# rogermm14/eonerf_code

Hardware: AMD Instinct MI355X
Metric: train rays/sec on JAX_068 (4096 rays x 128 samples) (higher is better)
Workload: dtype bf16

## Files before the change

eonerf_code_amd/csrc/eonerf_bwd_pipe.hip:

```cpp
#include "eonerf_common.h"
#include "eonerf_kernels.h"
#include "eonerf_ambient_dev.h"

namespace {

constexpr int NT = 512;
constexpr int TS = PIPE_TS;
constexpr int IMG_B = 16 * 1024;
constexpr int SLOT_B = 2 * IMG_B;
#ifndef EO_PIPE_STAMPS
#define EO_PIPE_STAMPS 0
#endif
constexpr int NSLOT = 4, DEPTH = 3, DDEPTH = 2;
static_assert(DDEPTH < DEPTH && DEPTH < NSLOT, "prefetch distances (the counted waits of Cnt assume DDEPTH < DEPTH)");
EO_DEV int slot_of(int k) { return k & (NSLOT - 1); }
constexpr uint32_t RING_USE = PIPE_RING;
constexpr int N_DMA = 4;
constexpr int CTRL_B = 64;
constexpr int SMEM_B = NSLOT * SLOT_B + CTRL_B;
constexpr int AUX_SC1 = 16, AUX_NT = 2;
constexpr unsigned long long WATCHDOG_TICKS = 30000000ull;

typedef __attribute__((address_space(1))) unsigned int gu32;

EO_DEV int wg_swz16(int row, int chunk) { return (chunk ^ ((row >> 2) & 3)) * 16; }

constexpr int NST = 2;
template <bool CTRL, bool ORDB> struct Cnt {
    static constexpr int C = (CTRL ? 4 : 0) + NST + N_DMA;
    static constexpr int TOP = ORDB ? C : N_DMA / 2 + (DDEPTH - 1) * C;
    static constexpr int TOP_CTRL = NST + N_DMA;
};

struct Stage {
    int pipe, st, n_k;
    bool has_in;
    int x_row;
    const uint8_t* in_lin;
    uint8_t* out_lin;
    bool local;
};

template <bool CTRL, int MODE, bool ORDB = false>
EO_DEV void run_stage(const BwdPipeArgs& a, const Stage& S, uint8_t* smem, int tid) {
    constexpr bool HAS_OUT = MODE == 0 || MODE == 1;
    constexpr bool RING_OUT = MODE == 0;
    typedef PBf16 P;
    typedef P::U U;
    const int lane = tid & 63, wave = __builtin_amdgcn_readfirstlane(tid >> 6), h = lane >> 5, c = lane & 31;
    int* const ctl = reinterpret_cast<int*>(smem + NSLOT * SLOT_B);
    const int n_k = S.n_k;

    U wt[16];
    {
        const uint8_t* src = a.wt + ((size_t)(S.st * 8 + wave) * 16) * 1024 + lane * 16;
#pragma unroll
        for (int kg = 0; kg < 16; ++kg) wt[kg] = *reinterpret_cast<const U*>(src + kg * 1024);
        __builtin_amdgcn_s_waitcnt(0x0F70);
    }
    f32x16 dw[8];
#pragma unroll
    for (int j = 0; j < 8; ++j) dw[j] = zero_acc();
    float db = 0.f;

    const size_t n_tiles = (size_t)a.p_pad / TS;
    const int n_edges = a.n_stages - 1;
    const uint8_t* x_base = reinterpret_cast<const uint8_t*>(a.act) + (size_t)S.x_row * n_tiles * SEG_B;
    uint8_t* const ring_in = a.rings + (size_t)(S.pipe * n_edges + (S.st - 1)) * PIPE_RING * IMG_B;
    uint8_t* const ring_out = a.rings + (size_t)(S.pipe * n_edges + S.st) * PIPE_RING * IMG_B;
    gu32* const f_in = (gu32*)(a.flags + (size_t)(S.pipe * n_edges + (S.st - 1)) * 64);
    gu32* const f_out = (gu32*)(a.flags + (size_t)(S.pipe * n_edges + S.st) * 64);
    gu32* const my_scratch = (gu32*)(a.scratch_word + (size_t)(S.pipe * a.n_stages + S.st) * 32);

    uint8_t* const grd_blk = S.out_lin;
    const uint8_t* const in_blk = S.in_lin;

    int x_voff[2];
#pragma unroll
    for (int j = 0; j < 2; ++j) {
        const int row = 32 * wave + 16 * j + (lane >> 2);
        x_voff[j] = row * SEG_B + (((lane & 3) ^ ((row >> 2) & 3)) * 16);
    }
    const uint32_t lin_stride = (uint32_t)a.n_pipes * IMG_B;
    const bool in_ring = S.has_in && !in_blk;
    const uint8_t* const d_base = !S.has_in ? a.dy_in + (size_t)S.pipe * IMG_B : (in_blk ? in_blk + (size_t)S.pipe * IMG_B : ring_in);
    const uint32_t d_mask = in_ring ? RING_USE - 1 : 0x7fffffffu, d_mul = in_ring ? IMG_B : lin_stride;
    const __amdgpu_buffer_rsrc_t rs_d = __builtin_amdgcn_make_buffer_rsrc(const_cast<uint8_t*>(d_base), 0, -1, 0x00020000);
    const __amdgpu_buffer_rsrc_t rs_x = __builtin_amdgcn_make_buffer_rsrc(const_cast<uint8_t*>(x_base) + (size_t)S.pipe * 256 * SEG_B, 0, -1, 0x00020000);
    const __amdgpu_buffer_rsrc_t rs_o = __builtin_amdgcn_make_buffer_rsrc(MODE == 0 ? ring_out : grd_blk + (size_t)S.pipe * IMG_B, 0, -1, 0x00020000);
    const int v_dy = lane * 16 + (2 * wave) * 1024;
    struct Dma { uint32_t so_d, so_x; uint8_t *slot, *slot_d; };
    auto dma_prep = [&](int kx, int kd) {
        Dma d;
        d.slot = smem + slot_of(kx) * SLOT_B;
        d.slot_d = smem + slot_of(kd) * SLOT_B;
        d.so_d = ((uint32_t)kd & d_mask) * d_mul;
        d.so_x = (uint32_t)kx * lin_stride;
        return d;
    };
    auto dma_piece = [&](const Dma& d, int i) {
        if (i < 2) {
            if (S.has_in)
                __builtin_amdgcn_raw_ptr_buffer_load_lds(rs_d, (__attribute__((address_space(3))) void*)(d.slot_d + (2 * wave + i) * 1024), 16,
                                                         lane * 16 + (2 * wave + i) * 1024, d.so_d, 0, AUX_SC1);
            else
                __builtin_amdgcn_raw_ptr_buffer_load_lds(rs_d, (__attribute__((address_space(3))) void*)(d.slot_d + (2 * wave + i) * 1024), 16,
                                                         lane * 16 + (2 * wave + i) * 1024, d.so_d, 0, AUX_NT);
        } else {
            __builtin_amdgcn_raw_ptr_buffer_load_lds(rs_x, (__attribute__((address_space(3))) void*)(d.slot + IMG_B + (32 * wave + 16 * (i - 2)) * SEG_B), 16,
                                                     x_voff[i - 2], d.so_x, 0, AUX_NT);
        }
    };
    auto issue = [&](int k, bool with_dy) {
        const Dma d = dma_prep(k, k);
#pragma unroll
        for (int i = 0; i < N_DMA; ++i) if (with_dy || i >= 2) dma_piece(d, i);
    };

    const int g4 = lane >> 4, i16 = lane & 15, qq = i16 >> 2, pp = i16 & 3;
    const int tr_off = (2 * wave + (g4 & 1)) * 1024 + ((pp & 1) * 32 + 8 * (g4 >> 1) + qq) * 16 + (pp >> 1) * 8;
    const int xb_off0 = IMG_B + c * SEG_B + wg_swz16(c, h), xb_off1 = IMG_B + c * SEG_B + wg_swz16(c, 2 + h);
    int xm_off[4];
#pragma unroll
    for (int q = 0; q < 4; ++q) {
        const int f0 = 32 * wave + 8 * q + 4 * (g4 >> 1);
        xm_off[q] = IMG_B + (f0 + qq) * SEG_B + wg_swz16(f0, 2 * (g4 & 1) + (pp >> 1)) + (pp & 1) * 8;
    }

    int known_head = S.has_in ? 0 : 0x7fffffff, known_tail = RING_OUT ? 0 : 0x7fffffff;
    unsigned ph = 0, pt = 0;
    auto poll_sync = [&](gu32* word) -> int {
        return (int)__hip_atomic_load(word, __ATOMIC_RELAXED, __HIP_MEMORY_SCOPE_AGENT);
    };
    bool aborted = false;
    auto wait_for = [&](gu32* word, int need, int& known) {
        if (known >= need || aborted) return;
        const unsigned long long t0 = __builtin_amdgcn_s_memrealtime();
        for (unsigned it = 0;; ++it) {
            known = poll_sync(word);
            if (known >= need) return;
            __builtin_amdgcn_s_sleep(2);
            const bool expired = __builtin_amdgcn_s_memrealtime() - t0 > WATCHDOG_TICKS;
            const bool other = (it & 63) == 63 && __hip_atomic_load(a.error, __ATOMIC_RELAXED, __HIP_MEMORY_SCOPE_AGENT) != 0;
            if (expired || other) {
                if (lane == 0) { if (expired) atomicOr(a.error, 1 << (S.st & 7)); ctl[0] = 1; }
                asm volatile("s_waitcnt lgkmcnt(0)" ::: "memory");
                aborted = true;
                return;
            }
        }
    };

    const bool stamp = EO_PIPE_STAMPS && a.stamps != nullptr;
    auto clk = [&]() -> uint32_t { return (uint32_t)__builtin_amdgcn_s_memtime(); };
    uint32_t t_slow = 0, t_top = 0, t_bar = 0, t_dx = 0, t_is = 0, t_dw = 0, n_slow = 0;
    const uint32_t t_begin = stamp ? clk() : 0;

    if (CTRL && S.has_in) wait_for(f_in, n_k < DDEPTH ? n_k : DDEPTH, known_head);
    if (CTRL) asm volatile("s_waitcnt vmcnt(0) lgkmcnt(0)" ::: "memory");
    __syncthreads();
    if (ctl[0]) return;
#pragma unroll
    for (int d = 0; d < DEPTH; ++d) issue(d < n_k ? d : n_k - 1, d < DDEPTH);
    asm volatile("s_waitcnt vmcnt(%0)" ::"n"((DEPTH - 1) * N_DMA - (DEPTH - DDEPTH) * (N_DMA / 2)) : "memory");

    for (int k = 0; k < n_k; ++k) {
        uint8_t* slot = smem + slot_of(k) * SLOT_B;
        const uint32_t tt0 = stamp ? clk() : 0;
        asm volatile("s_waitcnt vmcnt(%0)" ::"n"(CTRL ? Cnt<CTRL, ORDB>::TOP_CTRL : Cnt<CTRL, ORDB>::TOP) : "memory");
        const uint32_t tt1 = stamp ? clk() : 0;
        if (CTRL) {
            asm volatile("" : "+v"(ph), "+v"(pt));
            if (k >= 1) {
                const int vh = __builtin_amdgcn_readfirstlane((int)ph), vt = __builtin_amdgcn_readfirstlane((int)pt);
                if (S.has_in && vh > known_head) known_head = vh;
                if (RING_OUT && vt > known_tail) known_tail = vt;
            }
            const int need_in = k + DDEPTH < n_k ? k + DDEPTH + 1 : n_k;
            const int need_out = k + 1 - RING_USE;
            const uint32_t ts0 = stamp ? clk() : 0;
            const bool slow = (S.has_in && known_head < need_in) || (RING_OUT && known_tail < need_out);
            if (S.has_in && known_head < need_in) wait_for(f_in, need_in, known_head);
            if (RING_OUT && known_tail < need_out) wait_for(f_out + 32, need_out, known_tail);
            if (stamp && slow) { t_slow += clk() - ts0; ++n_slow; }
        }
        asm volatile("s_barrier" ::: "memory");
        const uint32_t tt2 = stamp ? clk() : 0;
        if (stamp) { t_top += tt1 - tt0; t_bar += tt2 - tt1; }
        if ((k & 7) == 0 && ctl[0]) return;
        if (CTRL) {
            if (lane == 0) {
                if (S.has_in) __hip_atomic_store(f_in + 32, (unsigned)(k + 1), __ATOMIC_RELAXED, __HIP_MEMORY_SCOPE_AGENT);
                else __hip_atomic_store(my_scratch, 0u, __ATOMIC_RELAXED, __HIP_MEMORY_SCOPE_AGENT);
                if (HAS_OUT) __hip_atomic_store(f_out, (unsigned)(k > 0 && S.st != a.fault_stage ? k - 1 : 0), __ATOMIC_RELAXED, __HIP_MEMORY_SCOPE_AGENT);
                else __hip_atomic_store((my_scratch + 1), 0u, __ATOMIC_RELAXED, __HIP_MEMORY_SCOPE_AGENT);
            }
            const gu32* a_h = S.has_in ? f_in : my_scratch;
            const gu32* a_t = RING_OUT ? f_out + 32 : my_scratch;
            asm volatile("global_load_dword %0, %2, off sc1\n\tglobal_load_dword %1, %3, off sc1"
                         : "=&v"(ph), "=&v"(pt) : "v"(a_h), "v"(a_t) : "memory");
        }

        auto phase_dx = [&]() {
            f32x16 acc = zero_acc();
            u32x2 xm[4] = {};
            {
                const uint8_t* bp = slot + lane * 16;
                constexpr int WIN = 3;
                U fr[WIN];
#pragma unroll
                for (int d = 0; d < WIN; ++d) fr[d] = lds_unit<P>(bp + d * 1024);
#pragma unroll
                for (int kg = 0; kg < 16; ++kg) {
                    acc = P::mma(wt[kg], fr[kg % WIN], acc);
                    if (kg + WIN < 16) fr[kg % WIN] = lds_unit<P>(bp + (kg + WIN) * 1024);
                    __builtin_amdgcn_sched_barrier(0);
                }
            }
            asm volatile("ds_read_b64_tr_b16 %0, %4\n\t"
                         "ds_read_b64_tr_b16 %1, %5\n\t"
                         "ds_read_b64_tr_b16 %2, %6\n\t"
                         "ds_read_b64_tr_b16 %3, %7\n\t"
                         "s_waitcnt lgkmcnt(0)"
                         : "=&v"(xm[0]), "=&v"(xm[1]), "=&v"(xm[2]), "=&v"(xm[3])
                         : "v"((uint32_t)(uintptr_t)(slot + xm_off[0])), "v"((uint32_t)(uintptr_t)(slot + xm_off[1])),
                           "v"((uint32_t)(uintptr_t)(slot + xm_off[2])), "v"((uint32_t)(uintptr_t)(slot + xm_off[3])) : "memory");
            uint32_t w8[8];
#pragma unroll
            for (int s = 0; s < 8; ++s) {
                uint32_t flags, r;
                const uint32_t xw = xm[s >> 1][s & 1];
                asm("v_pk_min_u16 %0, %1, %2" : "=v"(flags) : "v"(xw), "v"(0x00010001u));
                asm("v_pk_mul_lo_u16 %0, %1, %2" : "=v"(r) : "v"(cvt_pk_bf16(acc[2 * s], acc[2 * s + 1])), "v"(flags));
                w8[s] = r;
            }
            const uint32_t so_o = MODE == 0 ? ((uint32_t)k & (RING_USE - 1)) * IMG_B : (uint32_t)k * lin_stride;
            if (HAS_OUT && S.local) {
                __builtin_amdgcn_raw_buffer_store_b128(u32x4{w8[0], w8[1], w8[2], w8[3]}, rs_o, v_dy, so_o, 0);
                __builtin_amdgcn_raw_buffer_store_b128(u32x4{w8[4], w8[5], w8[6], w8[7]}, rs_o, v_dy + 1024, so_o, 0);
            } else if (HAS_OUT) {
                __builtin_amdgcn_raw_buffer_store_b128(u32x4{w8[0], w8[1], w8[2], w8[3]}, rs_o, v_dy, so_o, AUX_SC1);
                __builtin_amdgcn_raw_buffer_store_b128(u32x4{w8[4], w8[5], w8[6], w8[7]}, rs_o, v_dy + 1024, so_o, AUX_SC1);
            } else {
                __builtin_amdgcn_raw_buffer_store_b128(u32x4{w8[0], w8[1], w8[2], w8[3]}, rs_o, v_dy, so_o, AUX_NT);
                __builtin_amdgcn_raw_buffer_store_b128(u32x4{w8[4], w8[5], w8[6], w8[7]}, rs_o, v_dy + 1024, so_o, AUX_NT);
            }
        };
        u32x2 ta[2][2] = {};
        auto dw_prefetch = [&]() {
            const uint32_t ra = (uint32_t)(uintptr_t)(slot + tr_off);
            asm volatile("ds_read_b64_tr_b16 %0, %4\n\t"
                         "ds_read_b64_tr_b16 %1, %4 offset:64\n\t"
                         "ds_read_b64_tr_b16 %2, %4 offset:256\n\t"
                         "ds_read_b64_tr_b16 %3, %4 offset:320"
                         : "=&v"(ta[0][0]), "=&v"(ta[0][1]), "=&v"(ta[1][0]), "=&v"(ta[1][1]) : "v"(ra) : "memory");
        };
        auto phase_dw = [&]() {
            asm volatile("s_waitcnt lgkmcnt(0)" : "+v"(ta[0][0]), "+v"(ta[0][1]), "+v"(ta[1][0]), "+v"(ta[1][1]) :: "memory");
#pragma unroll
            for (int ks = 0; ks < 2; ++ks) {
                const U af = __builtin_bit_cast(U, u32x4{ta[ks][0][0], ta[ks][0][1], ta[ks][1][0], ta[ks][1][1]});
                const uint8_t* xb = slot + (ks ? xb_off1 : xb_off0);
                U bf[2];
                bf[0] = lds_unit<P>(xb);
                bf[1] = lds_unit<P>(xb + 2048);
#pragma unroll
                for (int j = 0; j < 8; ++j) {
                    dw[j] = P::mma(af, bf[j & 1], dw[j]);
                    if (j + 2 < 8) bf[j & 1] = lds_unit<P>(xb + (j + 2) * 2048);
                    __builtin_amdgcn_sched_barrier(0);
                }
                const u32x4 av = __builtin_bit_cast(u32x4, af);
#pragma unroll
                for (int e = 0; e < 4; ++e) db += __uint_as_float(av[e] << 16) + __uint_as_float(av[e] & 0xffff0000u);
            }
        };
        const int k_next = k + DEPTH < n_k ? k + DEPTH : n_k - 1;
        const Dma dma = dma_prep(k_next, k + DDEPTH < n_k ? k + DDEPTH : n_k - 1);
        auto issue_block = [&]() {
#pragma unroll
            for (int i = 0; i < N_DMA; ++i) dma_piece(dma, i);
        };
        if (!ORDB) {
            phase_dx();
            const uint32_t tt3 = stamp ? clk() : 0;
            dw_prefetch();
            issue_block();
            const uint32_t tt4 = stamp ? clk() : 0;
            phase_dw();
            if (stamp) { t_dx += tt3 - tt2; t_is += tt4 - tt3; t_dw += clk() - tt4; }
        } else {
            dw_prefetch();
            issue_block();
            const uint32_t tt3 = stamp ? clk() : 0;
            phase_dw();
            const uint32_t tt4 = stamp ? clk() : 0;
            phase_dx();
            if (stamp) { t_is += tt3 - tt2; t_dw += tt4 - tt3; t_dx += clk() - tt4; }
        }
    }
    if (stamp && lane == 0) {
        unsigned long long* o = a.stamps + ((size_t)(S.pipe * a.n_stages + S.st) * 8 + wave) * 16;
        o[0] = clk() - t_begin; o[1] = t_slow; o[2] = t_top; o[3] = t_bar; o[4] = t_dx; o[5] = n_slow; o[6] = (unsigned long long)n_k;
        o[7] = 0; o[8] = t_is; o[9] = 0; o[10] = t_dw;
    }
    asm volatile("s_waitcnt vmcnt(0)" ::: "memory");
    __syncthreads();
    if (CTRL && lane == 0 && HAS_OUT && S.st != a.fault_stage) __hip_atomic_store(f_out, (unsigned)n_k, __ATOMIC_RELAXED, __HIP_MEMORY_SCOPE_AGENT);

    db += __shfl_xor(db, 32, 64);
    if (a.partials) {
        float* pt = a.partials + (size_t)(S.pipe * a.n_stages + S.st) * (256 * 256 + 256);
#pragma unroll
        for (int j = 0; j < 8; ++j)
#pragma unroll
            for (int g = 0; g < 16; ++g) pt[(32 * wave + acc_row(g, h)) * 256 + 32 * j + c] = dw[j][g];
        if (h == 0) pt[256 * 256 + 32 * wave + c] = db;
        return;
    }
    float* dwp = a.d_flat + a.dw_off[S.st];
    float* dbp = a.d_flat + a.db_off[S.st];
    const int ld = a.dw_ld[S.st];
    const int row0 = 32 * wave;
#pragma unroll
    for (int j = 0; j < 8; ++j)
#pragma unroll
        for (int g = 0; g < 16; ++g) atomicAdd(dwp + (size_t)(row0 + acc_row(g, h)) * ld + 32 * j + c, dw[j][g]);
    if (h == 0) atomicAdd(dbp + row0 + c, db);
}

EO_DEV bool take_role(const BwdPipeArgs& a, uint8_t* smem, int tid, Stage& S, int& extra) {
    int* const ctl = reinterpret_cast<int*>(smem + NSLOT * SLOT_B);
    if (tid == 0) {
        ctl[0] = 0; ctl[2] = 0;
        if (!a.xcd_local) ctl[1] = atomicAdd(a.role_counter, 1);
        else {
            const int xcc = (int)(__builtin_amdgcn_s_getreg((3 << 11) | 20) & 7u);
            const int rx = atomicAdd(a.role_counter + 1 + xcc, 1);
// ... 109 lines not shown
```

eonerf_code_amd/csrc/eonerf_enc_pair.hip:

```cpp
#include "eonerf_common.h"
#include "eonerf_kernels.h"

namespace {

constexpr int NT = 512;
constexpr int IMG = 16 * 1024;
constexpr int ENC_B = ENC_SLOTS * SEG_B;
constexpr int SLOT_B = 2 * IMG + ENC_B;
constexpr int NS = 4, DEPTH = NS - 1;
constexpr int N_DMA = 9;
constexpr int GP_F = 4 * 32 * 4;
constexpr int SMEM_B = NS * SLOT_B + 2 * GP_F * (int)sizeof(float);

EO_DEV int swz16(int row, int chunk) { return (chunk ^ ((row >> 2) & 3)) * 16; }

EO_DEV void enc_waves(const EncPairArgs& a, uint8_t* smem, int lane, int wave, int t0, int t1, int n_pts) {
    typedef PBf16 P;
    typedef P::U U;
    const int h = lane >> 5, c = lane & 31;
    const int s_src = wave >> 1, mt = wave & 1;
    U wt[16];
#pragma unroll
    for (int kg = 0; kg < 16; ++kg) wt[kg] = *reinterpret_cast<const U*>(a.wt + ((size_t)((s_src * 2 + mt) * 16 + kg)) * 1024 + lane * 16);
    float* gp_lds = reinterpret_cast<float*>(smem + NS * SLOT_B);
    const float eoff = h ? EO_PI_2_F : 0.0f;
    auto load_pos = [&](int t, float& x, float& y, float& z) {
        const int p = t * 32 + c;
        const bool live = p < n_pts;
        x = live ? a.px[p] : 0.f; y = live ? a.py[p] : 0.f; z = live ? a.pz[p] : 0.f;
    };
    auto finish = [&](int t_prev, int par) {
        const int p = t_prev * 32 + c;
        if (h == 0 && p < n_pts) {
            const f32x4* g = reinterpret_cast<const f32x4*>(gp_lds + par * GP_F);
            f32x4 v = g[c];
#pragma unroll
            for (int w = 1; w < 4; ++w) { const f32x4 u = g[w * 32 + c]; v[0] += u[0]; v[1] += u[1]; v[2] += u[2]; }
            a.g_pos[p] = v[0]; a.g_pos[(size_t)a.p_pad + p] = v[1]; a.g_pos[2 * (size_t)a.p_pad + p] = v[2];
        }
    };
    float x, y, z;
    load_pos(t0, x, y, z);
    for (int t = t0; t < t1; ++t) {
        const int slot = (t - t0) & (NS - 1), par = (t - t0) & 1;
        asm volatile("s_barrier" ::: "memory");
        if (wave == 0 && t > t0) finish(t - 1, par ^ 1);
        const uint8_t* bp = smem + slot * SLOT_B + s_src * IMG + lane * 16;
        f32x16 acc = zero_acc();
        U fr[3];
#pragma unroll
        for (int d = 0; d < 3; ++d) fr[d] = lds_unit<P>(bp + d * 1024);
#pragma unroll
        for (int kg = 0; kg < 16; ++kg) {
            acc = P::mma(wt[kg], fr[kg % 3], acc);
            if (kg + 3 < 16) fr[kg % 3] = lds_unit<P>(bp + (kg + 3) * 1024);
        }
        float gp[3] = {0.f, 0.f, 0.f};
#pragma unroll
        for (int r = 0; r < 16; ++r) {
            const float g = acc[r];
            if (mt == 0 || r < 14) {
                const int q0 = r, q1 = 16 + r;
                const int k = mt ? q1 / 3 : q0 / 3, d = mt ? q1 % 3 : q0 % 3;
                const float cc = d == 0 ? x : (d == 1 ? y : z);
                const float arg = cc * (float)(1 << k) + eoff;
                gp[d] += g * (__cosf(arg) * (float)(1 << k));
            } else if (r == 14) {
                if (h) gp[2] += g; else gp[0] += g;
            } else {
                if (!h) gp[1] += g;
            }
        }
#pragma unroll
        for (int d = 0; d < 3; ++d) gp[d] += __shfl_xor(gp[d], 32, 64);
        if (h == 0) reinterpret_cast<f32x4*>(gp_lds + par * GP_F)[wave * 32 + c] = f32x4{gp[0], gp[1], gp[2], 0.f};
        if (t + 1 < t1) load_pos(t + 1, x, y, z);
    }
    asm volatile("s_barrier" ::: "memory");
    if (wave == 0) finish(t1 - 1, (t1 - 1 - t0) & 1);
}

EO_DEV void dw_waves(const EncPairArgs& a, uint8_t* smem, int lane, int wave, int t0, int t1) {
    typedef PBf16 P;
    typedef P::U U;
    const int h = lane >> 5, c = lane & 31, v = wave - 4;
    const int s_src = v >> 1, mhalf = v & 1;
    const size_t nt = (size_t)a.p_pad / 32;
    const uint8_t* grd = reinterpret_cast<const uint8_t*>(a.grd);
    const __amdgpu_buffer_rsrc_t rs_y0 = __builtin_amdgcn_make_buffer_rsrc(const_cast<uint8_t*>(grd) + (size_t)GRD_ROW_Y0 * nt * SEG_B, 0, -1, 0x00020000);
    const __amdgpu_buffer_rsrc_t rs_y5 = __builtin_amdgcn_make_buffer_rsrc(const_cast<uint8_t*>(grd) + (size_t)(GRD_ROW_Y0 + 5 * 256) * nt * SEG_B, 0, -1, 0x00020000);
    const __amdgpu_buffer_rsrc_t rs_e = __builtin_amdgcn_make_buffer_rsrc(const_cast<uint8_t*>(reinterpret_cast<const uint8_t*>(a.act)) + (size_t)ACT_ROW_ENC * nt * SEG_B, 0, -1, 0x00020000);
    const int enc_row = 16 * v + (lane >> 2);
    const int enc_voff = enc_row * SEG_B + (((lane & 3) ^ ((enc_row >> 2) & 3)) * 16);
    auto issue = [&](int t, int slot) {
        uint8_t* base = smem + slot * SLOT_B;
        const uint32_t so = (uint32_t)t * IMG;
#pragma unroll
        for (int i = 0; i < 4; ++i) {
            __builtin_amdgcn_raw_ptr_buffer_load_lds(rs_y0, (__attribute__((address_space(3))) void*)(base + (4 * v + i) * 1024), 16, lane * 16 + (4 * v + i) * 1024, so, 0, 2);
            __builtin_amdgcn_raw_ptr_buffer_load_lds(rs_y5, (__attribute__((address_space(3))) void*)(base + IMG + (4 * v + i) * 1024), 16, lane * 16 + (4 * v + i) * 1024, so, 0, 2);
        }
        __builtin_amdgcn_raw_ptr_buffer_load_lds(rs_e, (__attribute__((address_space(3))) void*)(base + 2 * IMG + 16 * v * SEG_B), 16, enc_voff, (uint32_t)t * ENC_B, 0, 2);
    };
    f32x16 dw[4][2];
    float dbv[4] = {0.f, 0.f, 0.f, 0.f};
#pragma unroll
    for (int i = 0; i < 4; ++i) { dw[i][0] = zero_acc(); dw[i][1] = zero_acc(); }
    const int g4 = lane >> 4, qq = (lane & 15) >> 2, pp = lane & 3;
    int off_a[4];
#pragma unroll
    for (int i = 0; i < 4; ++i)
        off_a[i] = s_src * IMG + (2 * (4 * mhalf + i) + (g4 & 1)) * 1024 + ((pp & 1) * 32 + 8 * (g4 >> 1) + qq) * 16 + (pp >> 1) * 8;
    int off_b[2][2];
#pragma unroll
    for (int j = 0; j < 2; ++j)
#pragma unroll
        for (int ks = 0; ks < 2; ++ks) { const int row = 32 * j + c; off_b[j][ks] = 2 * IMG + row * SEG_B + swz16(row, 2 * ks + h); }

#pragma unroll
    for (int d = 0; d < DEPTH; ++d) issue(t0 + d < t1 ? t0 + d : t1 - 1, d);
    for (int t = t0; t < t1; ++t) {
        const int slot = (t - t0) & (NS - 1);
        asm volatile("s_waitcnt vmcnt(%0)\n\ts_barrier" ::"n"(N_DMA * (DEPTH - 1)) : "memory");
        issue(t + DEPTH < t1 ? t + DEPTH : t1 - 1, (slot + DEPTH) & (NS - 1));
        const uint8_t* T = smem + slot * SLOT_B;
#pragma unroll
        for (int ks = 0; ks < 2; ++ks) {
            u32x2 ta[8];
            asm volatile("ds_read_b64_tr_b16 %0, %8\n\t"
                         "ds_read_b64_tr_b16 %1, %8 offset:64\n\t"
                         "ds_read_b64_tr_b16 %2, %9\n\t"
                         "ds_read_b64_tr_b16 %3, %9 offset:64\n\t"
                         "ds_read_b64_tr_b16 %4, %10\n\t"
                         "ds_read_b64_tr_b16 %5, %10 offset:64\n\t"
                         "ds_read_b64_tr_b16 %6, %11\n\t"
                         "ds_read_b64_tr_b16 %7, %11 offset:64\n\t"
                         "s_waitcnt lgkmcnt(0)"
                         : "=&v"(ta[0]), "=&v"(ta[1]), "=&v"(ta[2]), "=&v"(ta[3]), "=&v"(ta[4]), "=&v"(ta[5]), "=&v"(ta[6]), "=&v"(ta[7])
                         : "v"((uint32_t)(uintptr_t)(T + off_a[0] + 256 * ks)), "v"((uint32_t)(uintptr_t)(T + off_a[1] + 256 * ks)),
                           "v"((uint32_t)(uintptr_t)(T + off_a[2] + 256 * ks)), "v"((uint32_t)(uintptr_t)(T + off_a[3] + 256 * ks)) : "memory");
            const U b0 = lds_unit<P>(T + off_b[0][ks]), b1 = lds_unit<P>(T + off_b[1][ks]);
#pragma unroll
            for (int i = 0; i < 4; ++i) {
                const u32x4 av = u32x4{ta[2 * i][0], ta[2 * i][1], ta[2 * i + 1][0], ta[2 * i + 1][1]};
                const U af = __builtin_bit_cast(U, av);
                dw[i][0] = P::mma(af, b0, dw[i][0]);
                dw[i][1] = P::mma(af, b1, dw[i][1]);
                if (s_src == 0) {
#pragma unroll
                    for (int e = 0; e < 4; ++e) dbv[i] += __uint_as_float(av[e] << 16) + __uint_as_float(av[e] & 0xffff0000u);
                }
            }
        }
    }
    asm volatile("s_waitcnt vmcnt(0)" ::: "memory");
    float* part = a.part + (size_t)blockIdx.x * ENC_PART_F + (size_t)s_src * 256 * 64;
#pragma unroll
    for (int i = 0; i < 4; ++i)
#pragma unroll
        for (int j = 0; j < 2; ++j)
#pragma unroll
            for (int g = 0; g < 16; ++g) part[((4 * mhalf + i) * 32 + acc_row(g, h)) * 64 + 32 * j + c] = dw[i][j][g];
    if (s_src == 0) {
#pragma unroll
        for (int i = 0; i < 4; ++i) {
            const float sum = dbv[i] + __shfl_xor(dbv[i], 32, 64);
            if (h == 0) a.part[(size_t)blockIdx.x * ENC_PART_F + 2 * 256 * 64 + (4 * mhalf + i) * 32 + c] = sum;
        }
    }
}

__global__ __launch_bounds__(NT) void k_enc_pair(EncPairArgs a) {
    extern __shared__ __attribute__((aligned(16))) uint8_t smem[];
    const int lane = threadIdx.x & 63, wave = __builtin_amdgcn_readfirstlane(threadIdx.x >> 6);
    const int n_pts = *a.n_pts;
    const int n_tiles = (n_pts + 255) / 256 * 8;
    const int t0 = (int)((long long)blockIdx.x * n_tiles / gridDim.x), t1 = (int)((long long)(blockIdx.x + 1) * n_tiles / gridDim.x);
    if (t0 >= t1) {
        for (int i = threadIdx.x; i < ENC_PART_F; i += NT) a.part[(size_t)blockIdx.x * ENC_PART_F + i] = 0.f;
        return;
    }
    if (wave < 4) enc_waves(a, smem, lane, wave, t0, t1, n_pts);
    else dw_waves(a, smem, lane, wave, t0, t1);
}

}

hipError_t eo_launch_enc_pair(const EncPairArgs& a, int n_wg, hipStream_t st) {
    static EoAttrOnce attr;
    {
        const hipError_t e = attr.ensure([&] { return hipFuncSetAttribute(reinterpret_cast<const void*>(&k_enc_pair), hipFuncAttributeMaxDynamicSharedMemorySize, SMEM_B); });
        if (e != hipSuccess) return e;
    }
    hipLaunchKernelGGL(k_enc_pair, dim3(n_wg), dim3(NT), SMEM_B, st, a);
    return hipGetLastError();
}
```

eonerf_code_amd/csrc/eonerf_wgrad_dev.h:

```cpp
#pragma once
#include "eonerf_common.h"
#include "eonerf_kernels.h"
#include <type_traits>

namespace eo_wgrad {

constexpr int WG_NT = 512;
constexpr int MAX_ROWS = 256;
constexpr int ROW_B = SEG_B;
constexpr int OPND_B = MAX_ROWS * ROW_B;
constexpr int SLOT_B = 2 * OPND_B;
constexpr int NS = 4;
constexpr int DEPTH = NS - 1;
constexpr int WMAX = 4, NMAX = 2;
constexpr int AUX_B = 2048;
constexpr int AUX_SIG_WAVE = 7, AUX_EMB_WAVE = 6;

EO_DEV int wg_swz(int row, int chunk) { return (chunk ^ ((row >> 2) & 3)) * 16; }

constexpr int WG_SMEM = NS * SLOT_B + NS * AUX_B + 16;

template <class P>
EO_DEV void wgrad_work(const WgradJobTable& tab, int* queue, float* partials, uint8_t* smem) {
    typedef typename P::U U;
    constexpr int BK = ROW_B / P::ACT_BYTES;
    const int tid = threadIdx.x, lane = tid & 63, wid = __builtin_amdgcn_readfirstlane(tid >> 6), h = lane >> 5, r = lane & 31;
    uint8_t* const lds_aux = smem + NS * SLOT_B;
    int* const lds_item = reinterpret_cast<int*>(smem + NS * SLOT_B + NS * AUX_B);

  for (;;) {
    __syncthreads();
    if (tid == 0) *lds_item = atomicAdd(queue, 1);
    __syncthreads();
    const int item = __builtin_amdgcn_readfirstlane(*lds_item);
    if (item >= tab.items) return;
    int ji = 0;
    while (ji + 1 < tab.n && item >= tab.j[ji + 1].item0) ++ji;
    const WgradJob job = tab.j[ji];
    const int w = item - job.item0, n_slices = job.slices;
    const int n_pts = *job.n_pts;
    const int n_pad = (n_pts + P::TILE - 1) / P::TILE * P::TILE;
    const int steps = n_pad / BK;
    const int s0 = (int)((long long)w * steps / n_slices), s1 = (int)((long long)(w + 1) * steps / n_slices);
    if (s0 >= s1) continue;

    const int wm = job.wm, wn = job.wn, gn = job.gn;
    const bool active = wid < job.gm * gn;
    const int wm_idx = wid / gn, wn_idx = wid % gn;

    int voff_a[2], voff_b[2];
    bool on_a[2], on_b[2];
    int n_dma = 0;
#pragma unroll
    for (int j = 0; j < 2; ++j) {
        const int row = 32 * wid + 16 * j + (lane >> 2);
        const int chunk = (lane & 3) ^ ((row >> 2) & 3);
        const int ra = row < job.m_rows ? row : job.m_rows - 1, rb = row < job.n_rows ? row : job.n_rows - 1;
        voff_a[j] = job.a_units ? (32 * wid + 16 * j) * SEG_B + lane * 16 : ra * SEG_B + chunk * 16;
        voff_b[j] = rb * SEG_B + chunk * 16;
        on_a[j] = 32 * wid + 16 * j < job.m_rows;
        on_b[j] = 32 * wid + 16 * j < job.n_rows;
        n_dma += (on_a[j] ? 1 : 0) + (on_b[j] ? 1 : 0);
    }
    const bool has_aux = tab.aux.job == ji, has_sig = has_aux && tab.aux.a2 != nullptr, has_emb = has_aux && tab.aux.b2 != nullptr;
    const bool dma_sig = has_sig && wid == AUX_SIG_WAVE, dma_emb = has_emb && wid == AUX_EMB_WAVE;
    n_dma += (dma_sig ? 1 : 0) + (dma_emb ? 1 : 0);
    const __amdgpu_buffer_rsrc_t rs_a = __builtin_amdgcn_make_buffer_rsrc(const_cast<uint8_t*>(reinterpret_cast<const uint8_t*>(job.a)), 0, -1, 0x00020000);
    const __amdgpu_buffer_rsrc_t rs_b = __builtin_amdgcn_make_buffer_rsrc(const_cast<uint8_t*>(reinterpret_cast<const uint8_t*>(job.b)), 0, -1, 0x00020000);
    const __amdgpu_buffer_rsrc_t rs_a2 = __builtin_amdgcn_make_buffer_rsrc(const_cast<uint8_t*>(reinterpret_cast<const uint8_t*>(has_sig ? tab.aux.a2 : job.a)), 0, -1, 0x00020000);
    const __amdgpu_buffer_rsrc_t rs_b2 = __builtin_amdgcn_make_buffer_rsrc(const_cast<uint8_t*>(reinterpret_cast<const uint8_t*>(has_emb ? tab.aux.b2 : job.b)), 0, -1, 0x00020000);
    auto issue = [&](int step, int slot, auto aux_c) {
        if constexpr (decltype(aux_c)::value) {
        if (dma_sig) __builtin_amdgcn_raw_ptr_buffer_load_lds(rs_a2, (__attribute__((address_space(3))) void*)(lds_aux + slot * AUX_B), 16, lane * 16, (uint32_t)step * tab.aux.a2_stride, 0, 2);
        if (dma_emb) __builtin_amdgcn_raw_ptr_buffer_load_lds(rs_b2, (__attribute__((address_space(3))) void*)(lds_aux + slot * AUX_B + 1024), 16, lane * 16, (uint32_t)step * tab.aux.b2_stride, 0, 2);
        }
        uint8_t* base = smem + slot * SLOT_B + (32 * wid) * ROW_B;
        const uint32_t so_a = (uint32_t)step * job.a_stride, so_b = (uint32_t)step * job.b_stride;
#pragma unroll
        for (int j = 0; j < 2; ++j) {
            if (on_a[j]) __builtin_amdgcn_raw_ptr_buffer_load_lds(rs_a, (__attribute__((address_space(3))) void*)(base + 16 * j * ROW_B), 16, voff_a[j], so_a, 0, 2);
            if (on_b[j]) __builtin_amdgcn_raw_ptr_buffer_load_lds(rs_b, (__attribute__((address_space(3))) void*)(base + OPND_B + 16 * j * ROW_B), 16, voff_b[j], so_b, 0, 2);
        }
    };

    f32x16 acc[WMAX][NMAX];
    f32x16 accb = zero_acc();
#pragma unroll
    for (int i = 0; i < WMAX; ++i)
#pragma unroll
        for (int j = 0; j < NMAX; ++j) acc[i][j] = zero_acc();
    U ones = P::zero();
    if (r == 0) {
#pragma unroll
        for (int e = 0; e < P::NE; ++e) { if constexpr (P::IS_BF16) ones[e] = (__bf16)1.0f; else ones[e] = 1.0f; }
    }
    const bool do_bias = job.db != nullptr && active && wn_idx < wm;

    int off_a[WMAX][2], off_b[NMAX][2];
#pragma unroll
    for (int kg = 0; kg < 2; ++kg) {
#pragma unroll
        for (int i = 0; i < WMAX; ++i) {
            const int row = (wm_idx * wm + i) * 32 + r;
            off_a[i][kg] = row * ROW_B + wg_swz(row, 2 * kg + h);
            if (job.a_units) {
                const int g4 = lane >> 4, qq = (lane & 15) >> 2, pp = lane & 3;
                off_a[i][kg] = (2 * (wm_idx * wm + i) + (g4 & 1)) * 1024 + ((pp & 1) * 32 + 8 * (g4 >> 1) + qq) * 16 + (pp >> 1) * 8 + 256 * kg;
            }
        }
#pragma unroll
        for (int j = 0; j < NMAX; ++j) { const int row = (wn_idx * wn + j) * 32 + r; off_b[j][kg] = OPND_B + row * ROW_B + wg_swz(row, 2 * kg + h); }
    }

    struct SigRider { f32x16 acc; float b; };
    const bool sig_here = has_sig && wm_idx < wn;
    auto k_loop = [&](auto n_dma_c, auto units_c, auto aux_c, auto shape_c, SigRider* sr) {
        constexpr int N_DMA = decltype(n_dma_c)::value;
        constexpr bool UNITS = decltype(units_c)::value;
        constexpr bool AUX = decltype(aux_c)::value;
        constexpr int SHAPE = decltype(shape_c)::value;
        const int wm = SHAPE ? (SHAPE >> 4) : job.wm, wn = SHAPE ? (SHAPE & 15) : job.wn;
#pragma unroll
        for (int d = 0; d < DEPTH; ++d) issue(s0 + d < s1 ? s0 + d : s1 - 1, d, aux_c);
        for (int s = s0; s < s1; ++s) {
            const int slot = (s - s0) & (NS - 1);
            asm volatile("s_waitcnt vmcnt(%0)\n\ts_barrier" ::"n"(N_DMA * (DEPTH - 1)) : "memory");
            issue(s + DEPTH < s1 ? s + DEPTH : s1 - 1, (slot + DEPTH) & (NS - 1), aux_c);
            if (active) {
                const uint8_t* T = smem + slot * SLOT_B;
                if constexpr (UNITS) {
                    u32x2 t[8];
                    asm volatile("ds_read_b64_tr_b16 %0, %8\n\t"
                                 "ds_read_b64_tr_b16 %1, %8 offset:64\n\t"
                                 "ds_read_b64_tr_b16 %2, %9\n\t"
                                 "ds_read_b64_tr_b16 %3, %9 offset:64\n\t"
                                 "ds_read_b64_tr_b16 %4, %8 offset:256\n\t"
                                 "ds_read_b64_tr_b16 %5, %8 offset:320\n\t"
                                 "ds_read_b64_tr_b16 %6, %9 offset:256\n\t"
                                 "ds_read_b64_tr_b16 %7, %9 offset:320\n\t"
                                 "s_waitcnt lgkmcnt(0)"
                                 : "=&v"(t[0]), "=&v"(t[1]), "=&v"(t[2]), "=&v"(t[3]), "=&v"(t[4]), "=&v"(t[5]), "=&v"(t[6]), "=&v"(t[7])
                                 : "v"((uint32_t)(uintptr_t)(T + off_a[0][0])), "v"((uint32_t)(uintptr_t)(T + off_a[1][0])) : "memory");
#pragma unroll
                    for (int kg = 0; kg < 2; ++kg) {
                        const U bf0 = lds_unit<P>(T + off_b[0][kg]);
#pragma unroll
                        for (int i = 0; i < 2; ++i) {
                            const U af = __builtin_bit_cast(U, u32x4{t[4 * kg + 2 * i][0], t[4 * kg + 2 * i][1], t[4 * kg + 2 * i + 1][0], t[4 * kg + 2 * i + 1][1]});
                            acc[i][0] = P::mma(af, bf0, acc[i][0]);
                            if (do_bias && i == wn_idx) accb = P::mma(af, ones, accb);
                        }
                    }
                } else {
#pragma unroll
                for (int kg = 0; kg < 2; ++kg) {
                    U af[WMAX], bf[NMAX];
#pragma unroll
                    for (int i = 0; i < WMAX; ++i) if (i < wm) af[i] = lds_unit<P>(T + off_a[i][kg]);
#pragma unroll
                    for (int j = 0; j < NMAX; ++j) if (j < wn) bf[j] = lds_unit<P>(T + off_b[j][kg]);
                    U baux = ones;
                    if constexpr (AUX) {
                        const uint8_t* X = lds_aux + slot * AUX_B + (2 * kg + h) * 16;
                        if (has_emb && r >= 1 && r <= 4) baux = lds_unit<P>(X + 1024 + (r - 1) * ROW_B);
                        if (sig_here) {
                            U as = P::zero();
                            if (r == 0) as = lds_unit<P>(X);
                            sr->acc = P::mma(as, wm_idx == 0 ? bf[0] : bf[NMAX - 1], sr->acc);
                            if (wid == 0) {
#pragma unroll
                                for (int e = 0; e < P::NE; ++e) sr->b += (float)as[e];
                            }
                        }
                    }
#pragma unroll
                    for (int i = 0; i < WMAX; ++i)
                        if (i < wm) {
#pragma unroll
                            for (int j = 0; j < NMAX; ++j)
                                if (j < wn) acc[i][j] = P::mma(af[i], bf[j], acc[i][j]);
                            if (do_bias && i == wn_idx) accb = P::mma(af[i], baux, accb);
                        }
                }
                }
            }
        }
    };
    typedef std::integral_constant<bool, false> Rows;
    typedef std::integral_constant<bool, P::IS_BF16> Units;
    typedef std::integral_constant<bool, false> Plain;
    typedef std::integral_constant<bool, true> Riders;
    typedef std::integral_constant<int, 0> AnyShape;
#define EO_KL(N, U, A, S, SR) k_loop(std::integral_constant<int, N>(), U(), A(), std::integral_constant<int, S>(), SR)
    const int shape = 16 * wm + wn;
// ... 96 lines not shown
```

Baseline: 1.265 million.

## Pad and swizzle LDS unit layout for dY images to cut bank conflicts

Introduces a shared LDS layout header that pads each 1 KiB unit to a 1088-byte stride and XOR-swizzles the upper 32 chunks. The DMA sources, B-operand reads and transposed reads in the backward pipe, encoder pair and weight-grad kernels now use this layout. The aim is to remove LDS bank conflicts on the transposed ds_read_b64_tr_b16 and unit reads. In exchange each slot uses slightly more LDS, and the DMA source offsets get a per-lane permutation that must match the reader exactly.

```diff
diff --git a/eonerf_code_amd/csrc/eonerf_bwd_pipe.hip b/eonerf_code_amd/csrc/eonerf_bwd_pipe.hip
--- a/eonerf_code_amd/csrc/eonerf_bwd_pipe.hip
+++ b/eonerf_code_amd/csrc/eonerf_bwd_pipe.hip
@@ -1,13 +1,16 @@
 #include "eonerf_common.h"
 #include "eonerf_kernels.h"
 #include "eonerf_ambient_dev.h"
+#include "eonerf_lds_layout.h"
 
 namespace {
 
 constexpr int NT = 512;
 constexpr int TS = PIPE_TS;
 constexpr int IMG_B = 16 * 1024;
-constexpr int SLOT_B = 2 * IMG_B;
+constexpr int DIMG_B = eo_lds::image_bytes();
+constexpr int SLOT_B = DIMG_B + IMG_B;
+static_assert(DIMG_B % 16 == 0 && eo_lds::TILE_MEM_B == IMG_B, "the X image behind the dY image stays 16-byte aligned");
 #ifndef EO_PIPE_STAMPS
 #define EO_PIPE_STAMPS 0
 #endif
@@ -88,26 +91,28 @@
     const __amdgpu_buffer_rsrc_t rs_d = __builtin_amdgcn_make_buffer_rsrc(const_cast<uint8_t*>(d_base), 0, -1, 0x00020000);
     const __amdgpu_buffer_rsrc_t rs_x = __builtin_amdgcn_make_buffer_rsrc(const_cast<uint8_t*>(x_base) + (size_t)S.pipe * 256 * SEG_B, 0, -1, 0x00020000);
     const __amdgpu_buffer_rsrc_t rs_o = __builtin_amdgcn_make_buffer_rsrc(MODE == 0 ? ring_out : grd_blk + (size_t)S.pipe * IMG_B, 0, -1, 0x00020000);
-    const int v_dy = lane * 16 + (2 * wave) * 1024;
+    const int v_st = lane * 16, v_sw = eo_lds::dma_src_lane(lane);
+    static_assert(eo_lds::dma_src_lane(37) == eo_lds::b_lane(37), "one per-lane value serves the DMA source and the B-operand read");
+    const uint32_t s_unit = (uint32_t)eo_lds::dma_src_unit(2 * wave);
     struct Dma { uint32_t so_d, so_x; uint8_t *slot, *slot_d; };
     auto dma_prep = [&](int kx, int kd) {
         Dma d;
         d.slot = smem + slot_of(kx) * SLOT_B;
         d.slot_d = smem + slot_of(kd) * SLOT_B;
-        d.so_d = ((uint32_t)kd & d_mask) * d_mul;
+        d.so_d = ((uint32_t)kd & d_mask) * d_mul + s_unit;
         d.so_x = (uint32_t)kx * lin_stride;
         return d;
     };
     auto dma_piece = [&](const Dma& d, int i) {
         if (i < 2) {
             if (S.has_in)
-                __builtin_amdgcn_raw_ptr_buffer_load_lds(rs_d, (__attribute__((address_space(3))) void*)(d.slot_d + (2 * wave + i) * 1024), 16,
-                                                         lane * 16 + (2 * wave + i) * 1024, d.so_d, 0, AUX_SC1);
+                __builtin_amdgcn_raw_ptr_buffer_load_lds(rs_d, (__attribute__((address_space(3))) void*)(d.slot_d + eo_lds::dma_dst(2 * wave + i)), 16,
+                                                         v_sw, d.so_d + eo_lds::dma_src_unit(i), 0, AUX_SC1);
             else
-                __builtin_amdgcn_raw_ptr_buffer_load_lds(rs_d, (__attribute__((address_space(3))) void*)(d.slot_d + (2 * wave + i) * 1024), 16,
-                                                         lane * 16 + (2 * wave + i) * 1024, d.so_d, 0, AUX_NT);
+                __builtin_amdgcn_raw_ptr_buffer_load_lds(rs_d, (__attribute__((address_space(3))) void*)(d.slot_d + eo_lds::dma_dst(2 * wave + i)), 16,
+                                                         v_sw, d.so_d + eo_lds::dma_src_unit(i), 0, AUX_NT);
         } else {
-            __builtin_amdgcn_raw_ptr_buffer_load_lds(rs_x, (__attribute__((address_space(3))) void*)(d.slot + IMG_B + (32 * wave + 16 * (i - 2)) * SEG_B), 16,
+            __builtin_amdgcn_raw_ptr_buffer_load_lds(rs_x, (__attribute__((address_space(3))) void*)(d.slot + DIMG_B + (32 * wave + 16 * (i - 2)) * SEG_B), 16,
                                                      x_voff[i - 2], d.so_x, 0, AUX_NT);
         }
     };
@@ -118,13 +123,13 @@
     };
 
     const int g4 = lane >> 4, i16 = lane & 15, qq = i16 >> 2, pp = i16 & 3;
-    const int tr_off = (2 * wave + (g4 & 1)) * 1024 + ((pp & 1) * 32 + 8 * (g4 >> 1) + qq) * 16 + (pp >> 1) * 8;
-    const int xb_off0 = IMG_B + c * SEG_B + wg_swz16(c, h), xb_off1 = IMG_B + c * SEG_B + wg_swz16(c, 2 + h);
+    const int tr_off = eo_lds::tr_tile(wave) + eo_lds::tr_lane(lane);
+    const int xb_off0 = DIMG_B + c * SEG_B + wg_swz16(c, h), xb_off1 = DIMG_B + c * SEG_B + wg_swz16(c, 2 + h);
     int xm_off[4];
 #pragma unroll
     for (int q = 0; q < 4; ++q) {
         const int f0 = 32 * wave + 8 * q + 4 * (g4 >> 1);
-        xm_off[q] = IMG_B + (f0 + qq) * SEG_B + wg_swz16(f0, 2 * (g4 & 1) + (pp >> 1)) + (pp & 1) * 8;
+        xm_off[q] = DIMG_B + (f0 + qq) * SEG_B + wg_swz16(f0, 2 * (g4 & 1) + (pp >> 1)) + (pp & 1) * 8;
     }
 
     int known_head = S.has_in ? 0 : 0x7fffffff, known_tail = RING_OUT ? 0 : 0x7fffffff;
@@ -205,15 +210,15 @@
             f32x16 acc = zero_acc();
             u32x2 xm[4] = {};
             {
-                const uint8_t* bp = slot + lane * 16;
+                const uint8_t* bp = slot + v_sw;
                 constexpr int WIN = 3;
                 U fr[WIN];
 #pragma unroll
-                for (int d = 0; d < WIN; ++d) fr[d] = lds_unit<P>(bp + d * 1024);
+                for (int d = 0; d < WIN; ++d) fr[d] = lds_unit<P>(bp + eo_lds::b_unit(d));
 #pragma unroll
                 for (int kg = 0; kg < 16; ++kg) {
                     acc = P::mma(wt[kg], fr[kg % WIN], acc);
-                    if (kg + WIN < 16) fr[kg % WIN] = lds_unit<P>(bp + (kg + WIN) * 1024);
+                    if (kg + WIN < 16) fr[kg % WIN] = lds_unit<P>(bp + eo_lds::b_unit(kg + WIN));
                     __builtin_amdgcn_sched_barrier(0);
                 }
             }
@@ -234,26 +239,27 @@
                 asm("v_pk_mul_lo_u16 %0, %1, %2" : "=v"(r) : "v"(cvt_pk_bf16(acc[2 * s], acc[2 * s + 1])), "v"(flags));
                 w8[s] = r;
             }
-            const uint32_t so_o = MODE == 0 ? ((uint32_t)k & (RING_USE - 1)) * IMG_B : (uint32_t)k * lin_stride;
+            const uint32_t so_o = (MODE == 0 ? ((uint32_t)k & (RING_USE - 1)) * IMG_B : (uint32_t)k * lin_stride) + s_unit;
             if (HAS_OUT && S.local) {
-                __builtin_amdgcn_raw_buffer_store_b128(u32x4{w8[0], w8[1], w8[2], w8[3]}, rs_o, v_dy, so_o, 0);
-                __builtin_amdgcn_raw_buffer_store_b128(u32x4{w8[4], w8[5], w8[6], w8[7]}, rs_o, v_dy + 1024, so_o, 0);
+                __builtin_amdgcn_raw_buffer_store_b128(u32x4{w8[0], w8[1], w8[2], w8[3]}, rs_o, v_st, so_o, 0);
+                __builtin_amdgcn_raw_buffer_store_b128(u32x4{w8[4], w8[5], w8[6], w8[7]}, rs_o, v_st + 1024, so_o, 0);
             } else if (HAS_OUT) {
-                __builtin_amdgcn_raw_buffer_store_b128(u32x4{w8[0], w8[1], w8[2], w8[3]}, rs_o, v_dy, so_o, AUX_SC1);
-                __builtin_amdgcn_raw_buffer_store_b128(u32x4{w8[4], w8[5], w8[6], w8[7]}, rs_o, v_dy + 1024, so_o, AUX_SC1);
+                __builtin_amdgcn_raw_buffer_store_b128(u32x4{w8[0], w8[1], w8[2], w8[3]}, rs_o, v_st, so_o, AUX_SC1);
+                __builtin_amdgcn_raw_buffer_store_b128(u32x4{w8[4], w8[5], w8[6], w8[7]}, rs_o, v_st + 1024, so_o, AUX_SC1);
             } else {
-                __builtin_amdgcn_raw_buffer_store_b128(u32x4{w8[0], w8[1], w8[2], w8[3]}, rs_o, v_dy, so_o, AUX_NT);
-                __builtin_amdgcn_raw_buffer_store_b128(u32x4{w8[4], w8[5], w8[6], w8[7]}, rs_o, v_dy + 1024, so_o, AUX_NT);
+                __builtin_amdgcn_raw_buffer_store_b128(u32x4{w8[0], w8[1], w8[2], w8[3]}, rs_o, v_st, so_o, AUX_NT);
+                __builtin_amdgcn_raw_buffer_store_b128(u32x4{w8[4], w8[5], w8[6], w8[7]}, rs_o, v_st + 1024, so_o, AUX_NT);
             }
         };
         u32x2 ta[2][2] = {};
         auto dw_prefetch = [&]() {
             const uint32_t ra = (uint32_t)(uintptr_t)(slot + tr_off);
             asm volatile("ds_read_b64_tr_b16 %0, %4\n\t"
-                         "ds_read_b64_tr_b16 %1, %4 offset:64\n\t"
-                         "ds_read_b64_tr_b16 %2, %4 offset:256\n\t"
-                         "ds_read_b64_tr_b16 %3, %4 offset:320"
-                         : "=&v"(ta[0][0]), "=&v"(ta[0][1]), "=&v"(ta[1][0]), "=&v"(ta[1][1]) : "v"(ra) : "memory");
+                         "ds_read_b64_tr_b16 %1, %4 offset:%5\n\t"
+                         "ds_read_b64_tr_b16 %2, %4 offset:%6\n\t"
+                         "ds_read_b64_tr_b16 %3, %4 offset:%7"
+                         : "=&v"(ta[0][0]), "=&v"(ta[0][1]), "=&v"(ta[1][0]), "=&v"(ta[1][1])
+                         : "v"(ra), "n"(eo_lds::tr_imm(1, 0)), "n"(eo_lds::tr_imm(0, 1)), "n"(eo_lds::tr_imm(1, 1)) : "memory");
         };
         auto phase_dw = [&]() {
             asm volatile("s_waitcnt lgkmcnt(0)" : "+v"(ta[0][0]), "+v"(ta[0][1]), "+v"(ta[1][0]), "+v"(ta[1][1]) :: "memory");
diff --git a/eonerf_code_amd/csrc/eonerf_enc_pair.hip b/eonerf_code_amd/csrc/eonerf_enc_pair.hip
--- a/eonerf_code_amd/csrc/eonerf_enc_pair.hip
+++ b/eonerf_code_amd/csrc/eonerf_enc_pair.hip
@@ -1,16 +1,20 @@
 #include "eonerf_common.h"
 #include "eonerf_kernels.h"
+#include "eonerf_lds_layout.h"
 
 namespace {
 
 constexpr int NT = 512;
 constexpr int IMG = 16 * 1024;
+constexpr int LIMG = eo_lds::image_bytes();
 constexpr int ENC_B = ENC_SLOTS * SEG_B;
-constexpr int SLOT_B = 2 * IMG + ENC_B;
+constexpr int SLOT_B = 2 * LIMG + ENC_B;
+static_assert(eo_lds::TILE_MEM_B == IMG, "tile size");
 constexpr int NS = 4, DEPTH = NS - 1;
 constexpr int N_DMA = 9;
 constexpr int GP_F = 4 * 32 * 4;
 constexpr int SMEM_B = NS * SLOT_B + 2 * GP_F * (int)sizeof(float);
+static_assert(SMEM_B <= 160 * 1024, "one workgroup per CU");
 
 EO_DEV int swz16(int row, int chunk) { return (chunk ^ ((row >> 2) & 3)) * 16; }
 
@@ -45,15 +49,15 @@
         const int slot = (t - t0) & (NS - 1), par = (t - t0) & 1;
         asm volatile("s_barrier" ::: "memory");
         if (wave == 0 && t > t0) finish(t - 1, par ^ 1);
-        const uint8_t* bp = smem + slot * SLOT_B + s_src * IMG + lane * 16;
+        const uint8_t* bp = smem + slot * SLOT_B + s_src * LIMG + eo_lds::b_lane(lane);
         f32x16 acc = zero_acc();
         U fr[3];
 #pragma unroll
-        for (int d = 0; d < 3; ++d) fr[d] = lds_unit<P>(bp + d * 1024);
+        for (int d = 0; d < 3; ++d) fr[d] = lds_unit<P>(bp + eo_lds::b_unit(d));
 #pragma unroll
         for (int kg = 0; kg < 16; ++kg) {
             acc = P::mma(wt[kg], fr[kg % 3], acc);
-            if (kg + 3 < 16) fr[kg % 3] = lds_unit<P>(bp + (kg + 3) * 1024);
+            if (kg + 3 < 16) fr[kg % 3] = lds_unit<P>(bp + eo_lds::b_unit(kg + 3));
         }
         float gp[3] = {0.f, 0.f, 0.f};
 #pragma unroll
@@ -90,32 +94,32 @@
     const __amdgpu_buffer_rsrc_t rs_y0 = __builtin_amdgcn_make_buffer_rsrc(const_cast<uint8_t*>(grd) + (size_t)GRD_ROW_Y0 * nt * SEG_B, 0, -1, 0x00020000);
     const __amdgpu_buffer_rsrc_t rs_y5 = __builtin_amdgcn_make_buffer_rsrc(const_cast<uint8_t*>(grd) + (size_t)(GRD_ROW_Y0 + 5 * 256) * nt * SEG_B, 0, -1, 0x00020000);
     const __amdgpu_buffer_rsrc_t rs_e = __builtin_amdgcn_make_buffer_rsrc(const_cast<uint8_t*>(reinterpret_cast<const uint8_t*>(a.act)) + (size_t)ACT_ROW_ENC * nt * SEG_B, 0, -1, 0x00020000);
+    const int v_sw = eo_lds::dma_src_lane(lane);
     const int enc_row = 16 * v + (lane >> 2);
     const int enc_voff = enc_row * SEG_B + (((lane & 3) ^ ((enc_row >> 2) & 3)) * 16);
     auto issue = [&](int t, int slot) {
         uint8_t* base = smem + slot * SLOT_B;
-        const uint32_t so = (uint32_t)t * IMG;
+        const uint32_t so = (uint32_t)t * IMG + eo_lds::dma_src_unit(4 * v);
 #pragma unroll
         for (int i = 0; i < 4; ++i) {
-            __builtin_amdgcn_raw_ptr_buffer_load_lds(rs_y0, (__attribute__((address_space(3))) void*)(base + (4 * v + i) * 1024), 16, lane * 16 + (4 * v + i) * 1024, so, 0, 2);
-            __builtin_amdgcn_raw_ptr_buffer_load_lds(rs_y5, (__attribute__((address_space(3))) void*)(base + IMG + (4 * v + i) * 1024), 16, lane * 16 + (4 * v + i) * 1024, so, 0, 2);
-        }
-        __builtin_amdgcn_raw_ptr_buffer_load_lds(rs_e, (__attribute__((address_space(3))) void*)(base + 2 * IMG + 16 * v * SEG_B), 16, enc_voff, (uint32_t)t * ENC_B, 0, 2);
+            __builtin_amdgcn_raw_ptr_buffer_load_lds(rs_y0, (__attribute__((address_space(3))) void*)(base + eo_lds::dma_dst(4 * v + i)), 16, v_sw, so + eo_lds::dma_src_unit(i), 0, 2);
+            __builtin_amdgcn_raw_ptr_buffer_load_lds(rs_y5, (__attribute__((address_space(3))) void*)(base + LIMG + eo_lds::dma_dst(4 * v + i)), 16, v_sw, so + eo_lds::dma_src_unit(i), 0, 2);
+        }
+        __builtin_amdgcn_raw_ptr_buffer_load_lds(rs_e, (__attribute__((address_space(3))) void*)(base + 2 * LIMG + 16 * v * SEG_B), 16, enc_voff, (uint32_t)t * ENC_B, 0, 2);
     };
     f32x16 dw[4][2];
     float dbv[4] = {0.f, 0.f, 0.f, 0.f};
 #pragma unroll
     for (int i = 0; i < 4; ++i) { dw[i][0] = zero_acc(); dw[i][1] = zero_acc(); }
-    const int g4 = lane >> 4, qq = (lane & 15) >> 2, pp = lane & 3;
     int off_a[4];
 #pragma unroll
-    for (int i = 0; i < 4; ++i)
-        off_a[i] = s_src * IMG + (2 * (4 * mhalf + i) + (g4 & 1)) * 1024 + ((pp & 1) * 32 + 8 * (g4 >> 1) + qq) * 16 + (pp >> 1) * 8;
+    for (int i = 0; i < 4; ++i) off_a[i] = s_src * LIMG + eo_lds::tr_tile(4 * mhalf + i) + eo_lds::tr_lane(lane);
+    static_assert(eo_lds::tr_imm(1, 0) == 64 && eo_lds::tr_imm(0, 1) == 256, "the immediates of the reads below");
     int off_b[2][2];
 #pragma unroll
     for (int j = 0; j < 2; ++j)
 #pragma unroll
-        for (int ks = 0; ks < 2; ++ks) { const int row = 32 * j + c; off_b[j][ks] = 2 * IMG + row * SEG_B + swz16(row, 2 * ks + h); }
+        for (int ks = 0; ks < 2; ++ks) { const int row = 32 * j + c; off_b[j][ks] = 2 * LIMG + row * SEG_B + swz16(row, 2 * ks + h); }
 
 #pragma unroll
     for (int d = 0; d < DEPTH; ++d) issue(t0 + d < t1 ? t0 + d : t1 - 1, d);
diff --git a/eonerf_code_amd/csrc/eonerf_lds_layout.h b/eonerf_code_amd/csrc/eonerf_lds_layout.h
--- /dev/null
+++ b/eonerf_code_amd/csrc/eonerf_lds_layout.h
@@ -0,0 +1,38 @@
+#pragma once
+
+#if defined(__HIPCC__) || defined(__CUDACC__)
+#define EO_LDS_HD __host__ __device__
+#else
+#define EO_LDS_HD
+#endif
+
+namespace eo_lds {
+
+constexpr int UNITS = 16;
+constexpr int UNIT_B = 1024;
+constexpr int CHUNK_B = 16;
+constexpr int TILE_MEM_B = UNITS * UNIT_B;
+
+EO_LDS_HD constexpr int unit_stride() { return 1088; }
+EO_LDS_HD constexpr int chunk_swz(int c) { return c ^ (8 * ((c >> 5) & 1)); }
+EO_LDS_HD constexpr int image_bytes() { return UNITS * unit_stride(); }
+EO_LDS_HD constexpr int chunk_at(int u, int c) { return u * unit_stride() + chunk_swz(c) * CHUNK_B; }
+
+EO_LDS_HD constexpr int dma_dst(int u) { return u * unit_stride(); }
+EO_LDS_HD constexpr int dma_src_lane(int lane) { return chunk_swz(lane) * CHUNK_B; }
+EO_LDS_HD constexpr int dma_src_unit(int u) { return u * UNIT_B; }
+
+EO_LDS_HD constexpr int b_lane(int lane) { return chunk_swz(lane) * CHUNK_B; }
+EO_LDS_HD constexpr int b_unit(int kg) { return kg * unit_stride(); }
+
+EO_LDS_HD constexpr int tr_lane(int lane) {
+    const int g4 = lane >> 4, qq = (lane & 15) >> 2, pp = lane & 3;
+    return chunk_at(g4 & 1, (pp & 1) * 32 + 8 * (g4 >> 1) + qq) + (pp >> 1) * 8;
+}
+EO_LDS_HD constexpr int tr_tile(int mt) { return 2 * mt * unit_stride(); }
+EO_LDS_HD constexpr int tr_imm(int t, int ks) { return 64 * t + 256 * ks; }
+
+static_assert(unit_stride() % CHUNK_B == 0 && unit_stride() >= UNIT_B, "a unit is written as one 1-KiB LDS-DMA piece of 16-byte chunks");
+static_assert(chunk_swz(chunk_swz(45)) == 45 && chunk_swz(13) == 13 && chunk_swz(37) == 45, "the chunk swizzle is an involution on the upper 32 chunks");
+
+}
diff --git a/eonerf_code_amd/csrc/eonerf_wgrad_dev.h b/eonerf_code_amd/csrc/eonerf_wgrad_dev.h
--- a/eonerf_code_amd/csrc/eonerf_wgrad_dev.h
+++ b/eonerf_code_amd/csrc/eonerf_wgrad_dev.h
@@ -1,6 +1,7 @@
 #pragma once
 #include "eonerf_common.h"
 #include "eonerf_kernels.h"
+#include "eonerf_lds_layout.h"
 #include <type_traits>
 
 namespace eo_wgrad {
@@ -9,7 +10,9 @@
 constexpr int MAX_ROWS = 256;
 constexpr int ROW_B = SEG_B;
 constexpr int OPND_B = MAX_ROWS * ROW_B;
-constexpr int SLOT_B = 2 * OPND_B;
+constexpr int OPND_A_B = eo_lds::image_bytes();
+constexpr int SLOT_B = OPND_A_B + OPND_B;
+static_assert(OPND_A_B >= OPND_B && OPND_A_B % 16 == 0 && eo_lds::TILE_MEM_B == OPND_B, "row-order A tiles use the first 16 KiB");
 constexpr int NS = 4;
 constexpr int DEPTH = NS - 1;
 constexpr int WMAX = 4, NMAX = 2;
@@ -56,7 +59,7 @@
         const int row = 32 * wid + 16 * j + (lane >> 2);
         const int chunk = (lane & 3) ^ ((row >> 2) & 3);
         const int ra = row < job.m_rows ? row : job.m_rows - 1, rb = row < job.n_rows ? row : job.n_rows - 1;
-        voff_a[j] = job.a_units ? (32 * wid + 16 * j) * SEG_B + lane * 16 : ra * SEG_B + chunk * 16;
+        voff_a[j] = job.a_units ? eo_lds::dma_src_unit(2 * wid + j) + eo_lds::dma_src_lane(lane) : ra * SEG_B + chunk * 16;
         voff_b[j] = rb * SEG_B + chunk * 16;
         on_a[j] = 32 * wid + 16 * j < job.m_rows;
         on_b[j] = 32 * wid + 16 * j < job.n_rows;
@@ -75,11 +78,12 @@
         if (dma_emb) __builtin_amdgcn_raw_ptr_buffer_load_lds(rs_b2, (__attribute__((address_space(3))) void*)(lds_aux + slot * AUX_B + 1024), 16, lane * 16, (uint32_t)step * tab.aux.b2_stride, 0, 2);
         }
         uint8_t* base = smem + slot * SLOT_B + (32 * wid) * ROW_B;
+        uint8_t* base_u = smem + slot * SLOT_B + eo_lds::dma_dst(2 * wid);
         const uint32_t so_a = (uint32_t)step * job.a_stride, so_b = (uint32_t)step * job.b_stride;
 #pragma unroll
         for (int j = 0; j < 2; ++j) {
-            if (on_a[j]) __builtin_amdgcn_raw_ptr_buffer_load_lds(rs_a, (__attribute__((address_space(3))) void*)(base + 16 * j * ROW_B), 16, voff_a[j], so_a, 0, 2);
-            if (on_b[j]) __builtin_amdgcn_raw_ptr_buffer_load_lds(rs_b, (__attribute__((address_space(3))) void*)(base + OPND_B + 16 * j * ROW_B), 16, voff_b[j], so_b, 0, 2);
+            if (on_a[j]) __builtin_amdgcn_raw_ptr_buffer_load_lds(rs_a, (__attribute__((address_space(3))) void*)(job.a_units ? base_u + eo_lds::dma_dst(j) : base + 16 * j * ROW_B), 16, voff_a[j], so_a, 0, 2);
+            if (on_b[j]) __builtin_amdgcn_raw_ptr_buffer_load_lds(rs_b, (__attribute__((address_space(3))) void*)(base + OPND_A_B + 16 * j * ROW_B), 16, voff_b[j], so_b, 0, 2);
         }
     };
 
@@ -104,12 +108,11 @@
             const int row = (wm_idx * wm + i) * 32 + r;
             off_a[i][kg] = row * ROW_B + wg_swz(row, 2 * kg + h);
             if (job.a_units) {
-                const int g4 = lane >> 4, qq = (lane & 15) >> 2, pp = lane & 3;
-                off_a[i][kg] = (2 * (wm_idx * wm + i) + (g4 & 1)) * 1024 + ((pp & 1) * 32 + 8 * (g4 >> 1) + qq) * 16 + (pp >> 1) * 8 + 256 * kg;
-            }
-        }
-#pragma unroll
-        for (int j = 0; j < NMAX; ++j) { const int row = (wn_idx * wn + j) * 32 + r; off_b[j][kg] = OPND_B + row * ROW_B + wg_swz(row, 2 * kg + h); }
+                off_a[i][kg] = eo_lds::tr_tile(wm_idx * wm + i) + eo_lds::tr_lane(lane) + eo_lds::tr_imm(0, kg);
+            }
+        }
+#pragma unroll
+        for (int j = 0; j < NMAX; ++j) { const int row = (wn_idx * wn + j) * 32 + r; off_b[j][kg] = OPND_A_B + row * ROW_B + wg_swz(row, 2 * kg + h); }
     }
 
     struct SigRider { f32x16 acc; float b; };
```

Result: no change. 1.264 million, median of 2 (-0.1%).
